# CompVis/unsupervised-part-segmentation

Measured on AMD Instinct MI355X. Metric: images/sec training (CUB 128x128, 10 parts), higher is better.
Workload: dtype bf16

## Files before the change

unsupervised-part-segmentation_amd/csrc/conv_wgrad.hip:

```cpp
#include "common.h"

namespace {

struct WgK {
    int n, hi, wi, ci, ldi, ci_log, cin_v, ho, wo, co, ldo, in_sy, in_sx, ntaps, act_in, want_bias, in_f16;
    float act_slope;
    unsigned long long tap_off, tap_wi;
    const void* in; const void* dout; float* ws;
    float* bias_direct;
};

__device__ inline int wtap_dy(unsigned long long off, int t) { return (int)((off >> (4 * t + 2)) & 3) - 1; }
__device__ inline int wtap_dx(unsigned long long off, int t) { return (int)((off >> (4 * t)) & 3) - 1; }
__device__ inline int wtap_w(unsigned long long wi, int t) { return (int)((wi >> (4 * t)) & 15); }

constexpr int lds_stride(int row_bytes) {
    return ((row_bytes + 63) / 128) * 128 + 64;
}

typedef __attribute__((address_space(3))) s16x4 lds_s16x4;

__device__ inline bf16x8 tr_frag(const unsigned char* tile, int rs, int k0, int c0, int lane) {
    const int g = lane >> 4, i = lane & 15, h = g >> 1;
    const int cb = c0 + 16 * (g & 1), q = i >> 2, pp = i & 3;
    const unsigned char* a0 = tile + (k0 + 8 * h + q) * rs + (cb + 4 * pp) * 2;
    s16x4 lo = __builtin_amdgcn_ds_read_tr16_b64_v4i16((lds_s16x4*)a0);
    s16x4 hi = __builtin_amdgcn_ds_read_tr16_b64_v4i16((lds_s16x4*)(a0 + 4 * rs));
    union { s16x4 s[2]; bf16x8 b; } u;
    u.s[0] = lo; u.s[1] = hi;
    return u.b;
}

template <typename T, int BMW, int BNW>
__global__ __launch_bounds__(256) void conv_wgrad_kernel(const WgK p, const int M, const int cit, const int cot,
                                                         const int chunks_total, const int chunks_per) {
    constexpr int EPC = Chunk<T>::N;
    constexpr int PK = 4 * EPC;
    constexpr int RSA = lds_stride(BMW * (int)sizeof(T));
    constexpr int RSB = lds_stride(BNW * (int)sizeof(T));
    constexpr int NBM = BMW / 32, NBN = BNW / 32;
    constexpr int WM = NBM >= 2 ? ((NBN == 1 && NBM == 4) ? 4 : 2) : 1;
    constexpr int WN = NBN >= 2 ? ((NBM == 1 && NBN == 4) ? 4 : 2) : 1;
    constexpr int TM = NBM / WM, TN = NBN / WN;
    constexpr int ACTIVE = WM * WN;
    constexpr int CPA = BMW / EPC;
    constexpr int CPB = BNW / EPC;
    constexpr int NA = (PK * CPA + 255) / 256;
    constexpr int NB = (PK * CPB + 255) / 256;
    constexpr int BPARTS = 256 / BNW;

    __shared__ __attribute__((aligned(16))) unsigned char smem[PK * (RSA + RSB)];
    unsigned char* Xs = smem;
    unsigned char* Ds = smem + PK * RSA;

    const int tid = threadIdx.x, lane = tid & 63, wid = tid >> 6;
    const float act_ns = ups_slope_eff(p.act_in, p.act_slope);
    const int cot_i = blockIdx.x % cot, cit_i = blockIdx.x / cot;
    const int split = blockIdx.y;
    const int wm = wid / WN, wn = wid % WN;

    const T* __restrict__ in = (const T*)p.in;
    const T* __restrict__ dout = (const T*)p.dout;
    const int hw_o = p.ho * p.wo;
    const int V = p.ntaps * p.ci;
    const int v0 = cit_i * BMW, co0 = cot_i * BNW;
    const bool do_bias = p.want_bias && cit_i == 0;

    const int c_begin = split * chunks_per;
    const int c_end = min(chunks_total, c_begin + chunks_per);

    int xrow0 = 0, xrow1 = 0, xc0 = -1, xc1 = -1, xdy0 = 0, xdx0 = 0, xdy1 = 0, xdx1 = 0;
    {
        auto dec = [&](int idx, int& row, int& c, int& dy, int& dx) {
            c = -1;
            if (idx < PK * CPA) {
                row = idx / CPA;
                const int v = v0 + (idx - row * CPA) * EPC;
                if (v < V) {
                    const int tap = v / p.ci;
                    c = v - tap * p.ci;
                    dy = wtap_dy(p.tap_off, tap); dx = wtap_dx(p.tap_off, tap);
                }
            }
        };
        dec(tid, xrow0, xc0, xdy0, xdx0);
        if (NA > 1) dec(tid + 256, xrow1, xc1, xdy1, xdx1);
    }

    uint4 xa0, xa1, db0, db1;
    const uint4 zero4 = make_uint4(0u, 0u, 0u, 0u);

    auto load_x = [&](int chunk_idx, int row, int c, int dy, int dx) -> uint4 {
        uint4 v = zero4;
        const int m = chunk_idx * PK + row;
        if (c >= 0 && m < M) {
            const int img = m / hw_o, rem = m - img * hw_o;
            const int i = rem / p.wo, j = rem - i * p.wo;
            const int y = i * p.in_sy + dy, x = j * p.in_sx + dx;
            if ((unsigned)y < (unsigned)p.hi && (unsigned)x < (unsigned)p.wi)
                v = *(const uint4*)(in + (((long long)img * p.hi + y) * p.wi + x) * p.ldi + c);
        }
        return v;
    };
    auto load_d = [&](int chunk_idx, int idx) -> uint4 {
        uint4 v = zero4;
        if (idx < PK * CPB) {
            const int row = idx / CPB, cc = idx - row * CPB;
            const int m = chunk_idx * PK + row;
            const int ch = co0 + cc * EPC;
            if (m < M && ch < p.ldo) v = *(const uint4*)(dout + (long long)m * p.ldo + ch);
        }
        return v;
    };
    auto act_u4 = [&](uint4 u) -> uint4 {
        if constexpr (__is_same(T, bf16)) {
            if (p.in_f16) return ups_act_chunk_f16_to_bf16(u, act_ns, p.act_in != UPS_ACT_NONE);
        }
        if (p.act_in != UPS_ACT_NONE) {
            u = ups_act_chunk(u, act_ns, (T*)nullptr);
        }
        return u;
    };
    auto load_chunk = [&](int chunk_idx) {
        xa0 = load_x(chunk_idx, xrow0, xc0, xdy0, xdx0);
        if (NA > 1) xa1 = load_x(chunk_idx, xrow1, xc1, xdy1, xdx1);
        db0 = load_d(chunk_idx, tid);
        if (NB > 1) db1 = load_d(chunk_idx, tid + 256);
    };
    auto stage_chunk = [&]() {
        if (tid < PK * CPA) { const int row = tid / CPA, cc = tid - row * CPA; *(uint4*)(Xs + row * RSA + cc * 16) = act_u4(xa0); }
        if (NA > 1) { const int idx = tid + 256, row = idx / CPA, cc = idx - row * CPA; *(uint4*)(Xs + row * RSA + cc * 16) = act_u4(xa1); }
        if (tid < PK * CPB) { const int row = tid / CPB, cc = tid - row * CPB; *(uint4*)(Ds + row * RSB + cc * 16) = db0; }
        if (NB > 1) { const int idx = tid + 256, row = idx / CPB, cc = idx - row * CPB; *(uint4*)(Ds + row * RSB + cc * 16) = db1; }
    };

    f32x16 acc[TM][TN];
#pragma unroll
    for (int i = 0; i < TM; ++i)
#pragma unroll
        for (int j = 0; j < TN; ++j)
#pragma unroll
            for (int e = 0; e < 16; ++e) acc[i][j][e] = 0.f;
    float bsum = 0.f;
    const int bcol = tid % BNW, bpart = tid / BNW;

    if (c_begin < c_end) load_chunk(c_begin);
    for (int c = c_begin; c < c_end; ++c) {
        stage_chunk();
        __syncthreads();
        if (c + 1 < c_end) load_chunk(c + 1);
        if (do_bias) {
#pragma unroll
            for (int k = 0; k < PK / BPARTS; ++k)
                bsum += ld_as_float<T>((const T*)(Ds + (bpart * (PK / BPARTS) + k) * RSB) + bcol);
        }
        if (wid < ACTIVE) {
            if constexpr (sizeof(T) == 2) {
#pragma unroll
                for (int ks = 0; ks < 2; ++ks) {
                    bf16x8 a[TM], bb[TN];
#pragma unroll
                    for (int i = 0; i < TM; ++i) a[i] = tr_frag(Xs, RSA, ks * 16, (wm * TM + i) * 32, lane);
#pragma unroll
                    for (int j = 0; j < TN; ++j) bb[j] = tr_frag(Ds, RSB, ks * 16, (wn * TN + j) * 32, lane);
#pragma unroll
                    for (int i = 0; i < TM; ++i)
#pragma unroll
                        for (int j = 0; j < TN; ++j)
                            acc[i][j] = __builtin_amdgcn_mfma_f32_32x32x16_bf16(a[i], bb[j], acc[i][j], 0, 0, 0);
                }
            } else {
                const int r = lane & 31, h = lane >> 5;
#pragma unroll
                for (int kk = 0; kk < 8; ++kk) {
                    float a[TM], bb[TN];
#pragma unroll
                    for (int i = 0; i < TM; ++i) a[i] = *(const float*)(Xs + (8 * h + kk) * RSA + ((wm * TM + i) * 32 + r) * 4);
#pragma unroll
                    for (int j = 0; j < TN; ++j) bb[j] = *(const float*)(Ds + (8 * h + kk) * RSB + ((wn * TN + j) * 32 + r) * 4);
#pragma unroll
                    for (int i = 0; i < TM; ++i)
#pragma unroll
                        for (int j = 0; j < TN; ++j)
                            acc[i][j] = __builtin_amdgcn_mfma_f32_32x32x2f32(a[i], bb[j], acc[i][j], 0, 0, 0);
                }
            }
        }
        __syncthreads();
    }

    const long long slab_sz = (long long)p.ntaps * p.cin_v * p.co + p.co;
    float* slab = p.ws + (long long)split * slab_sz;
    if (wid < ACTIVE) {
#pragma unroll
        for (int tn = 0; tn < TN; ++tn) {
            const int col = co0 + (wn * TN + tn) * 32 + (lane & 31);
            if (col >= p.co) continue;
#pragma unroll
            for (int tm = 0; tm < TM; ++tm)
#pragma unroll
                for (int e = 0; e < 16; ++e) {
                    const int v = v0 + (wm * TM + tm) * 32 + (e & 3) + 8 * (e >> 2) + 4 * (lane >> 5);
                    if (v < V) {
                        const int tap = v / p.ci, cch = v - tap * p.ci;
                        if (cch < p.ci_log)
                            slab[((long long)wtap_w(p.tap_wi, tap) * p.cin_v + cch) * p.co + col] = acc[tm][tn][e];
                    }
                }
        }
    }
    if (do_bias) {
        float* red = (float*)smem;
        red[tid] = bsum;
        __syncthreads();
        if (tid < BNW && co0 + tid < p.co) {
            float s = 0.f;
#pragma unroll
            for (int k = 0; k < BPARTS; ++k) s += red[k * BNW + tid];
            if (p.bias_direct) p.bias_direct[co0 + tid] = s;
            else slab[(long long)p.ntaps * p.cin_v * p.co + co0 + tid] = s;
        }
    }
}

__global__ __launch_bounds__(256) void wgrad_reduce_kernel(const float* __restrict__ ws, float* __restrict__ grad,
                                                           float* __restrict__ gbias, int splitk, int ntaps_w, int cin_v,
                                                           int ci_log, int co, long long slab) {
    __shared__ float red[8][32];
    const long long nw = (long long)ntaps_w * ci_log * co;
    const long long total = nw + (gbias ? co : 0);
    const int o = threadIdx.x & 31, g = threadIdx.x >> 5;
    for (long long base = (long long)blockIdx.x * 32; base < total; base += (long long)gridDim.x * 32) {
        const long long idx = base + o;
        const bool ok = idx < total;
        long long off = 0;
        float* dst = nullptr;
        if (ok) {
            if (idx < nw) {
                const int c = (int)(idx % co);
                const long long tr = idx / co;
                const int row = (int)(tr % ci_log), tap = (int)(tr / ci_log);
                off = ((long long)tap * cin_v + row) * co + c;
                dst = grad + off;
            } else {
                off = (long long)ntaps_w * cin_v * co + (idx - nw);
                dst = gbias + (idx - nw);
            }
        }
        float s0 = 0.f, s1 = 0.f, s2 = 0.f, s3 = 0.f;
        if (ok) {
            int k = g;
            for (; k + 24 < splitk; k += 32) {
                s0 += ws[(long long)k * slab + off]; s1 += ws[(long long)(k + 8) * slab + off];
                s2 += ws[(long long)(k + 16) * slab + off]; s3 += ws[(long long)(k + 24) * slab + off];
            }
            for (; k < splitk; k += 8) s0 += ws[(long long)k * slab + off];
        }
        red[g][o] = (s0 + s1) + (s2 + s3);
        __syncthreads();
        if (g == 0 && ok) {
            float t = red[0][o];
#pragma unroll
            for (int q = 1; q < 8; ++q) t += red[q][o];
            *dst = t;
        }
        __syncthreads();
    }
}

template <typename T, int BMW, int BNW>
void launch_tile(const WgK& k, int M, int splitk, hipStream_t s) {
    constexpr int PK = 4 * Chunk<T>::N;
    const int cit = ups_cdiv(k.ntaps * k.ci, BMW), cot = ups_cdiv(k.co, BNW);
    const int chunks_total = ups_cdiv(M, PK);
    const int chunks_per = ups_cdiv(chunks_total, splitk);
    hipLaunchKernelGGL((conv_wgrad_kernel<T, BMW, BNW>), dim3(cit * cot, splitk), dim3(256), 0, s, k, M, cit, cot,
                       chunks_total, chunks_per);
}

template <typename T, int BMW>
void launch_n(const WgK& k, int M, int splitk, hipStream_t s) {
    if (k.co > 64) launch_tile<T, BMW, 128>(k, M, splitk, s);
    else if (k.co > 32) launch_tile<T, BMW, 64>(k, M, splitk, s);
    else launch_tile<T, BMW, 32>(k, M, splitk, s);
}

int tile_of(int c) { return c > 64 ? 128 : (c > 32 ? 64 : 32); }

template <typename T>
void launch_m(const WgK& k, int M, int splitk, hipStream_t s) {
    const int bm = tile_of(k.ntaps * k.ci);
    if (bm == 128) launch_n<T, 128>(k, M, splitk, s);
    else if (bm == 64) launch_n<T, 64>(k, M, splitk, s);
    else launch_n<T, 32>(k, M, splitk, s);
}

int plan_splitk(const ups_wgrad_desc* d) {
    const long long M = (long long)d->n * d->ho * d->wo;
    const int pk = d->dtype == UPS_BF16 ? 32 : 16;
    const int v = d->ntaps * d->ci;
    const int tiles = ups_cdiv(v, tile_of(v)) * ups_cdiv(d->co, tile_of(d->co));
    const int chunks = ups_cdiv(M, pk);
    int sk = ups_cdiv(2048, tiles);
    const int max_by_work = chunks / 8 > 0 ? chunks / 8 : 1;
    if (sk > max_by_work) sk = max_by_work;
    if (sk > 512) sk = 512;
    if (sk < 1) sk = 1;
    return sk;
}

}

int ups_wgrad3x3_plan(const ups_wgrad_desc* d, int* splitk, int* slabs);
int ups_wgrad3x3_run(const ups_wgrad_desc* d, hipStream_t s);
int ups_wgrad3x3_f8_plan(const ups_wgrad_desc* d, int* splitk, int* slabs);
int ups_wgrad3x3_f8_run(const ups_wgrad_desc* d, hipStream_t s);

extern "C" int ups_conv_wgrad_plan(const ups_wgrad_desc* d, int32_t* splitk, size_t* workspace_bytes) {
    UPS_CHECK_ARG(d && splitk && workspace_bytes);
    UPS_CHECK_ARG(d->ntaps >= 1 && d->ntaps <= 9 && d->ci > 0 && d->co > 0);
    int sk3 = 0, slabs3 = 0;
    if (ups_wgrad3x3_f8_plan(d, &sk3, &slabs3) == 0 ||
        ups_wgrad3x3_plan(d, &sk3, &slabs3) == 0) {
        *splitk = sk3;
        *workspace_bytes = (size_t)slabs3 * ((size_t)d->ntaps * d->cin_v * d->co + d->co) * sizeof(float);
        return UPS_OK;
    }
    const int sk = plan_splitk(d);
    *splitk = sk;
    *workspace_bytes = (size_t)sk * ((size_t)d->ntaps * d->cin_v * d->co + d->co) * sizeof(float);
    return UPS_OK;
}

extern "C" int ups_conv_wgrad(const ups_wgrad_desc* d, void* stream) {
    UPS_CHECK_ARG(d != nullptr);
    UPS_CHECK_ARG(d->dtype == UPS_F32 || d->dtype == UPS_BF16);
    UPS_CHECK_ARG(d->in && d->dout && d->grad && d->workspace);
    UPS_CHECK_ARG(d->ci > 0 && d->ci % 8 == 0 && d->ldi % 8 == 0 && d->ci <= d->ldi && d->ldo % 8 == 0);
    UPS_CHECK_ARG(d->ci_log >= 1 && d->ci_log <= d->ci && d->cin_v >= d->ci_log);
    UPS_CHECK_ARG(d->ntaps >= 1 && d->ntaps <= 9 && d->splitk >= 1);
    UPS_CHECK_ARG(d->act_slope >= 0.f && d->act_slope <= 1.f);
    UPS_CHECK_ARG(((uintptr_t)d->in & 15) == 0 && ((uintptr_t)d->dout & 15) == 0);
    const long long M = (long long)d->n * d->ho * d->wo;
    UPS_CHECK_ARG(M > 0 && M <= 0x7fffffffLL);
    WgK k;
    k.n = d->n; k.hi = d->hi; k.wi = d->wi; k.ci = d->ci; k.ldi = d->ldi; k.ci_log = d->ci_log; k.cin_v = d->cin_v;
    k.ho = d->ho; k.wo = d->wo; k.co = d->co; k.ldo = d->ldo; k.in_sy = d->in_sy; k.in_sx = d->in_sx;
    k.ntaps = d->ntaps; k.act_in = d->act_in; k.act_slope = d->act_slope; k.want_bias = d->grad_bias != nullptr;
    k.in_f16 = d->in_f16;
    UPS_CHECK_ARG(!d->in_f16 || (d->dtype == UPS_BF16 && !d->mask_bits));
    k.in = d->in; k.dout = d->dout; k.ws = d->workspace; k.bias_direct = nullptr;
    k.tap_off = 0; k.tap_wi = 0;
    int max_tw = 0;
    for (int t = 0; t < d->ntaps; ++t) {
        UPS_CHECK_ARG(d->tap_dy[t] >= -1 && d->tap_dy[t] <= 2 && d->tap_dx[t] >= -1 && d->tap_dx[t] <= 2);
        UPS_CHECK_ARG(d->tap_w[t] >= 0 && d->tap_w[t] <= 15);
        k.tap_off |= (unsigned long long)(((d->tap_dy[t] + 1) << 2) | (d->tap_dx[t] + 1)) << (4 * t);
        k.tap_wi |= (unsigned long long)d->tap_w[t] << (4 * t);
        if (d->tap_w[t] > max_tw) max_tw = d->tap_w[t];
    }
    UPS_CHECK_ARG(max_tw < d->ntaps);
    hipStream_t s = (hipStream_t)stream;
    int nslabs = d->splitk;
    int sk3 = 0, slabs3 = 0;
    if (d->mask_bits) {
        UPS_CHECK_ARG(d->mask_batch > 0 && d->n % d->mask_batch == 0 && d->n / d->mask_batch <= 32);
        if (ups_wgrad3x3_plan(d, &sk3, &slabs3) != 0) {
            ups_set_error("ups_conv_wgrad: the part-masked form needs the bf16 3x3 / stride-1 patch kernel (16-aligned images)");
            return UPS_E_UNSUPPORTED;
        }
    }
    if (ups_wgrad3x3_f8_plan(d, &sk3, &slabs3) == 0) {
        UPS_CHECK_ARG(d->splitk == sk3 && d->dout_f8_scale && d->in_f8_scale && ((uintptr_t)d->dout_f8 & 15) == 0);
        if (ups_wgrad3x3_f8_run(d, s) != UPS_OK) { ups_set_error("ups_conv_wgrad: fp8 kernel launch setup failed"); return UPS_E_LAUNCH; }
        nslabs = slabs3;
    } else if (ups_wgrad3x3_plan(d, &sk3, &slabs3) == 0) {
        UPS_CHECK_ARG(d->splitk == sk3);
        if (ups_wgrad3x3_run(d, s) != UPS_OK) { ups_set_error("ups_conv_wgrad: patch kernel launch setup failed"); return UPS_E_LAUNCH; }
        nslabs = slabs3;
    } else {
        static int direct = -1;
        if (direct < 0) { const char* e = getenv("UPS_WGRAD_DIRECT"); direct = (e && e[0] == '0') ? 0 : 1; }
        const bool one = direct && d->splitk == 1;
        if (one) { k.ws = d->grad; k.bias_direct = d->grad_bias; }
        if (d->dtype == UPS_F32) launch_m<float>(k, (int)M, d->splitk, s);
        else launch_m<bf16>(k, (int)M, d->splitk, s);
        UPS_LAUNCH_CHECK();
        if (one) return UPS_OK;
    }
    UPS_LAUNCH_CHECK();
    const long long slab = (long long)d->ntaps * d->cin_v * d->co + d->co;
    const long long total = (long long)d->ntaps * d->ci_log * d->co + d->co;
    hipLaunchKernelGGL(wgrad_reduce_kernel, dim3(ups_cdiv(total, 32) > 8192 ? 8192 : ups_cdiv(total, 32)), dim3(256), 0,
                       s, d->workspace, d->grad, d->grad_bias, nslabs, d->ntaps, d->cin_v, d->ci_log, d->co, slab);
    UPS_LAUNCH_CHECK();
    return UPS_OK;
}
```

unsupervised-part-segmentation_amd/switches.py:

```python
import os
from collections import OrderedDict

SWITCHES = OrderedDict([
    ("UPS_LIB", ("", "ab", "lib.py", "path of the library to load instead of csrc/libupsparts_hip.so (A/B builds: tools/ab_build.sh)")),
    ("UPS_DIST_BACKEND", ("nccl", "product", "runner.py", "torch.distributed backend (nccl = RCCL; gloo for the CPU / one-GPU tests)")),
    ("UPS_GRAPH", ("0", "product", "model.py", "1: HIP-graph replay of the step (config key hip_graph)")),
    ("UPS_STREAM_PLAN", ("auto", "product", "model.py", "full | compact | auto: side-stream budget (config key stream_plan; DESIGN section 7)")),
    ("UPS_NO_OVERLAP", ("0", "ab", "ops.py", "1: everything on one stream (per-kernel profiles without CU sharing)")),
    ("UPS_POST_ACT", ("1", "ab", "nets.py", "0: activation-on-load everywhere instead of post-activation storage (config key post_activation_storage)")),
    ("UPS_SIGN_BITS", ("1", "ab", "ops.py", "0: input gradients read the forward input for act' instead of the producer's sign bytes")),
    ("UPS_VGG_FP8", ("0", "ab", "model.py", "1: fp8 copies through the perceptual trunk (config key vgg_fp8; measured slower, DESIGN 3b)")),
    ("UPS_F8_WGRAD", ("1", "ab", "ops.py", "0: bf16 weight gradients in precision fp8")),
    ("UPS_F8_PRODUCER", ("1", "ab", "ops.py", "0: fp8 copies converted by a separate pass instead of the producing epilogue")),
    ("UPS_TOWERS", ("1", "ab", "ops.py", "0: the critics' towers through the generic convolution path instead of the grouped launches")),
    ("UPS_STATE_KERNEL", ("1", "ab", "model.py", "0: the Lagrangian / EMA state update as ~30 torch launches instead of one kernel")),
    ("UPS_LATE_JOIN", ("1", "ab", "model.py", "0: a single rank joins the weight-gradient stream at every segment boundary")),
    ("UPS_EARLY_ADAM", ("1", "ab", "model.py", "0: every key's Adam at the end of the step instead of behind its weight gradients")),
    ("UPS_EARLY_ALPHA", ("1", "ab", "model.py", "0: the appearance code after the pose encoder instead of beside it on `aux`")),
    ("UPS_CRITIC_STREAMS", ("1", "ab", "model.py", "0: the three critics on one stream")),
    ("UPS_COORD_STREAM", ("1", "ab", "ops.py", "0: the CoordConv rows of the weight gradients on the weight-gradient stream itself")),
    ("UPS_NO_D2S", ("0", "ab", "ops.py", "1: the stride-2 layers' input gradient as four phase launches instead of one depth-to-space launch")),
    ("UPS_DP_SIDE_LAUNCH", ("1", "ab", "model.py", "0: bucket all-reduces launched from the launching stream (it then waits for the weight gradients)")),
    ("UPS_DP_STANDIN", ("0", "debug", "dist.py", "1: every bucket all-reduce replaced by a device copy on its own stream (one-GPU stream-budget probe)")),
    ("UPS_FORCE_COLLECTIVES", ("0", "test", "dist.py", "1: issue the collectives at world size 1 (the RCCL call pattern test)")),
    ("UPS_JOIN_TIMING", ("0", "debug", "model.py", "1: HIP events around the end-of-backward joins (tools/probes/join_wait.py)")),
    ("UPS_ROWS_KERNEL", ("1", "test", "conv3x3_rows.hip", "0: row-stream layers through the patch / generic kernels; force: also at small batches (parity tests)")),
    ("UPS_S2_KERNEL", ("1", "ab", "conv3x3_s2.hip", "0: the other stride-2 forwards through the generic kernel")),
    ("UPS_THIN_SW", ("32", "ab", "conv3x3_rows.hip", "16: 16-column strips in the logit convolution (measured equal)")),
    ("UPS_FIRST_LAYER", ("1", "ab", "conv3x3_first.hip", "0: the 3-channel first layers through the generic kernel")),
    ("UPS_FORCE_GENERIC_CONV", ("0", "test", "conv_igemm.hip", "1: every convolution through the generic gather kernel")),
    ("UPS_IGEMM_FORCE", ("", "test", "conv_igemm.hip", "tile variant of the generic kernel")),
    ("UPS_NO_SPLITK", ("0", "ab", "conv_igemm.hip", "1: no split-K for the small-grid generic launches")),
    ("UPS_NO_SMALL_PATCH", ("0", "ab", "conv3x3_patch.hip", "1: no small-tile patch instances")),
    ("UPS_PATCH_CST", ("", "ab", "conv3x3_patch.hip", "patch kernel: constant-stride instances on / off")),
    ("UPS_PATCH_DMA", ("1", "ab", "conv3x3_patch.hip", "0: register-staged patches instead of LDS-DMA")),
    ("UPS_PATCH_MID", ("", "ab", "conv3x3_patch.hip", "patch kernel: mid-size tile selection")),
    ("UPS_PATCH_OCC", ("", "ab", "conv3x3_patch.hip", "patch kernel: blocks per CU override")),
    ("UPS_PATCH_RAGGED", ("1", "ab", "conv3x3_patch.hip", "0: images that are not a multiple of 16 leave the patch kernel")),
    ("UPS_PATCH_STATIC", ("", "ab", "conv3x3_patch.hip", "patch kernel: static-geometry instances on / off")),
    ("UPS_PATCH_THIN128", ("", "ab", "conv3x3_patch.hip", "patch kernel: thin 128-wide instance selection")),
    ("UPS_PATCH_THINOUT", ("", "ab", "conv3x3_patch.hip", "patch kernel: thin-output instance selection")),
    ("UPS_RES_PATCH", ("1", "ab", "conv3x3_patch.hip", "0: the forward's residual from global memory instead of the resident patch")),
    ("UPS_RES_PATCH_DGRAD", ("1", "ab", "conv3x3_patch.hip", "0: the input gradient's residual and sign bytes fetched in the epilogue instead of from the resident patch (round 6)")),
    ("UPS_F8_SCALED", ("1", "ab", "conv3x3_patch.hip", "0: K = 32 fp8 MFMA instead of the block-scaled K = 128 form")),
    ("UPS_WGRAD_DIRECT", ("1", "ab", "conv_wgrad.hip", "0: single-split weight gradients through a slab + reduce launch")),
    ("UPS_WGRAD_SLIDE", ("1", "ab", "conv_wgrad3x3.hip", "0: the plain form of the 3x3 weight gradient (3 % slower step)")),
    ("UPS_PRIOR_PX", ("1", "ab", "priors.hip", "0: the staged prior kernels at P = 10 instead of the pixel-per-lane rings")),
    ("UPS_PRIOR_PX_BPI", ("", "test", "priors.hip", "cap on blocks per image of the pixel-per-lane prior kernels (multi-tile loops at three images)")),
    ("UPS_PRIOR_DIRECT", ("1", "ab", "priors.hip", "0: the staged prior kernels at P = 16 / 20 / 25 instead of the chunk-per-lane direct-from-global forms (round 6)")),
    ("UPS_SOFTMAX_PX", ("1", "ab", "partpath.hip", "0: the LDS-walking soft-max kernel at P = 10")),
    ("UPS_MOMENTS_PX", ("1", "ab", "partpath.hip", "0: the slab form of the spatial moments at P = 10")),
    ("UPS_MOMENTS_PX_BLOCKS", ("", "test", "partpath.hip", "blocks of the pixel-per-lane moments kernel")),
    ("UPS_UNPOOL_MFMA", ("1", "test", "partpath.hip", "0: the VALU form of unpool_bwd (the unit test compares both)")),
])

COMPILE_TIME = ("UPS_ABLATE_BARRIER", "UPS_ABLATE_PATCHWAIT", "UPS_ABLATE_WWAIT", "UPS_EPI_PRIO", "UPS_ABLATE_DMA", "UPS_ABLATE_EPI", "UPS_ABLATE_GLOAD", "UPS_ABLATE_LSTORE", "UPS_ABLATE_MFMA", "UPS_F8S_WN1", "UPS_OCC2_FRAG2",
                "UPS_PATCH_A2", "UPS_PHASE_TIMING", "UPS_W8_NO_DMA", "UPS_W8_NO_MFMA", "UPS_W8_NO_QUANT", "UPS_W8_NO_XLOAD", "UPS_WGRAD_NO_PIPE",
                "UPS_ROWS_FWD_SIGN", "UPS_ROWS_NO_FENCE", "UPS_VMAX_BUILTIN")
NOT_SWITCHES = ("UPS_ABI_VERSION", "UPS_ACT_", "UPS_OK", "UPS_E_", "UPS_BF16", "UPS_F16", "UPS_F32", "UPS_CHECK_ARG", "UPS_LAUNCH_CHECK")


def value(name):
    return os.environ.get(name, SWITCHES[name][0])


def flag(name):
    d = SWITCHES[name][0]
    v = os.environ.get(name, d)
    return v != "0" if d == "1" else v == "1"


def report():
    diff = ["{}={}".format(k, os.environ[k]) for k, (d, _, _, _) in SWITCHES.items() if k in os.environ and os.environ[k] != d]
    return "UPS switches: " + (", ".join(diff) if diff else "all defaults")
```

Baseline: 2108.

## Add phase-split LDS patch kernel for stride-2 3x3 weight gradients

Adds a dedicated weight-gradient kernel for 3x3 stride-2 bf16 convolutions. It stages a polyphase-decomposed input patch and a swizzled dout tile in double-buffered LDS, reads them with transpose reads, and feeds 32x32x16 MFMAs, with each wave covering three taps. This replaces the generic split-K kernel for those layers and is meant to cut redundant global loads and im2col overhead. The kernel is limited to narrow outputs (co <= 64, wo <= 64) and can be disabled with a new switch.

Result: no change. 2117 (median of 6 runs) (+0.4%).

```diff
diff --git a/unsupervised-part-segmentation_amd/csrc/conv_wgrad.hip b/unsupervised-part-segmentation_amd/csrc/conv_wgrad.hip
--- a/unsupervised-part-segmentation_amd/csrc/conv_wgrad.hip
+++ b/unsupervised-part-segmentation_amd/csrc/conv_wgrad.hip
@@ -315,6 +315,8 @@
 int ups_wgrad3x3_run(const ups_wgrad_desc* d, hipStream_t s);
 int ups_wgrad3x3_f8_plan(const ups_wgrad_desc* d, int* splitk, int* slabs);
 int ups_wgrad3x3_f8_run(const ups_wgrad_desc* d, hipStream_t s);
+bool ups_wgrad3x3_s2_eligible(const ups_wgrad_desc* d);
+int ups_wgrad3x3_s2_run(const ups_wgrad_desc* d, float* ws, float* bias_direct, hipStream_t s);
 
 extern "C" int ups_conv_wgrad_plan(const ups_wgrad_desc* d, int32_t* splitk, size_t* workspace_bytes) {
     UPS_CHECK_ARG(d && splitk && workspace_bytes);
@@ -383,7 +385,12 @@
         if (direct < 0) { const char* e = getenv("UPS_WGRAD_DIRECT"); direct = (e && e[0] == '0') ? 0 : 1; }
         const bool one = direct && d->splitk == 1;
         if (one) { k.ws = d->grad; k.bias_direct = d->grad_bias; }
-        if (d->dtype == UPS_F32) launch_m<float>(k, (int)M, d->splitk, s);
+        if (ups_wgrad3x3_s2_eligible(d)) {
+            if (ups_wgrad3x3_s2_run(d, k.ws, k.bias_direct, s) != UPS_OK) {
+                ups_set_error("ups_conv_wgrad: stride-2 patch kernel launch setup failed");
+                return UPS_E_LAUNCH;
+            }
+        } else if (d->dtype == UPS_F32) launch_m<float>(k, (int)M, d->splitk, s);
         else launch_m<bf16>(k, (int)M, d->splitk, s);
         UPS_LAUNCH_CHECK();
         if (one) return UPS_OK;
diff --git a/unsupervised-part-segmentation_amd/csrc/conv_wgrad3x3_s2.hip b/unsupervised-part-segmentation_amd/csrc/conv_wgrad3x3_s2.hip
--- /dev/null
+++ b/unsupervised-part-segmentation_amd/csrc/conv_wgrad3x3_s2.hip
@@ -0,0 +1,274 @@
+#include <stdlib.h>
+
+#include "common.h"
+
+namespace {
+
+constexpr int CB = 32;
+constexpr int RSX = 64;
+constexpr int PK = 32;
+
+struct WgS2K {
+    int hi, wi, ho, wo, ci, ldi, ci_log, cin_v, co, ldo, act_in, want_bias, in_f16;
+    int M, chunks_per, th, plc, plp;
+    float act_slope;
+    int trow[9];
+    unsigned long long tap_wi;
+    const void* in; const void* dout; float* ws;
+    float* bias_direct;
+};
+
+typedef __attribute__((address_space(3))) s16x4 lds_s2_s16x4;
+
+__device__ inline bf16x8 tr_frag_x(const unsigned char* tile, int row0, int lane) {
+    const int g = lane >> 4, i = lane & 15, h = g >> 1;
+    const int cb = 16 * (g & 1), q = i >> 2, pp = i & 3;
+    const unsigned char* a0 = tile + (row0 + 8 * h + q) * RSX + (cb + 4 * pp) * 2;
+    s16x4 lo = __builtin_amdgcn_ds_read_tr16_b64_v4i16((lds_s2_s16x4*)a0);
+    s16x4 hi = __builtin_amdgcn_ds_read_tr16_b64_v4i16((lds_s2_s16x4*)(a0 + 4 * RSX));
+    union { s16x4 s[2]; bf16x8 b; } u;
+    u.s[0] = lo; u.s[1] = hi;
+    return u.b;
+}
+
+template <int BN> __device__ __forceinline__ int ds_swz(int row) {
+    if constexpr (BN == 64) return (row >> 1) & 1;
+    else return 0;
+}
+template <int BN> __device__ __forceinline__ int d_off(int row, int col) {
+    return row * (BN * 2) + (((col >> 5) ^ ds_swz<BN>(row)) << 6) + (col & 31) * 2;
+}
+
+template <int BN>
+__device__ inline bf16x8 tr_frag_dout(const unsigned char* tile, int row0, int wco, int lane) {
+    constexpr int RS = BN * 2;
+    const int g = lane >> 4, i = lane & 15, h = g >> 1, q = i >> 2, pp = i & 3;
+    const int row = row0 + 8 * h + q;
+    const unsigned char* a0 = tile + row * RS + ((wco ^ ds_swz<BN>(row)) << 6) + 32 * (g & 1) + 8 * pp;
+    s16x4 lo = __builtin_amdgcn_ds_read_tr16_b64_v4i16((lds_s2_s16x4*)a0);
+    s16x4 hi = __builtin_amdgcn_ds_read_tr16_b64_v4i16((lds_s2_s16x4*)(a0 + 4 * RS));
+    union { s16x4 s[2]; bf16x8 b; } u;
+    u.s[0] = lo; u.s[1] = hi;
+    return u.b;
+}
+
+template <int BN> struct S2Geo {
+    static constexpr int WCO = BN / 32;
+    static constexpr int NWC = 3 * WCO;
+    static constexpr int NW = NWC < 4 ? 4 : NWC;
+    static constexpr int NT = 64 * NW;
+    static constexpr int SPX = 128;
+    static constexpr int XMAX = 4 * 3 * 65;
+    static constexpr int NX = (XMAX * 4 + NT - 1) / NT;
+    static constexpr int ND = (SPX * BN / 8 + NT - 1) / NT;
+    static constexpr int XB = XMAX * RSX, DB = SPX * BN * 2;
+    static constexpr int BPARTS = 256 / BN;
+};
+
+template <int BN>
+__global__ __launch_bounds__(S2Geo<BN>::NT) void conv_wgrad3x3_s2_kernel(const WgS2K p, const int cot) {
+    using G = S2Geo<BN>;
+    constexpr int NT = G::NT, NX = G::NX, ND = G::ND, SPX = G::SPX, CPD = BN / 8;
+    extern __shared__ __attribute__((aligned(16))) unsigned char smem[];
+    unsigned char* Xbuf = smem;
+    unsigned char* Dbuf = smem + 2 * G::XB;
+
+    const int tid = threadIdx.x, lane = tid & 63;
+    const int wid = __builtin_amdgcn_readfirstlane(tid >> 6);
+    const float act_ns = ups_slope_eff(p.act_in, p.act_slope);
+    const int cot_i = blockIdx.x % cot, cit_i = blockIdx.x / cot, split = blockIdx.y;
+    const int ci0 = cit_i * CB, co0 = cot_i * BN;
+    const bf16* __restrict__ in = (const bf16*)p.in;
+    const bf16* __restrict__ dout = (const bf16*)p.dout;
+    const bool do_bias = p.want_bias && cit_i == 0;
+    const bool cwave = wid < G::NWC;
+    const int w_co = wid % G::WCO, w_t0 = 3 * (wid / G::WCO);
+
+    const int m_beg = split * p.chunks_per * PK;
+    const int m_end = min(p.M, m_beg + p.chunks_per * PK);
+    const int hw_o = p.ho * p.wo;
+    const int st_beg = m_beg / SPX, st_end = m_beg < m_end ? (m_end + SPX - 1) / SPX : st_beg;
+
+    const int nxi = 4 * p.plp * 4;
+    unsigned xrc[NX], xs[NX];
+#pragma unroll
+    for (int k = 0; k < NX; ++k) {
+        const int item = min(tid + NT * k, nxi - 1);
+        const int pix = item >> 2, cc = item & 3;
+        const int pl = pix / p.plp, rem = pix - pl * p.plp;
+        const int a = rem / p.plc, b = rem - a * p.plc;
+        const int r = 2 * a + (pl >> 1), c = 2 * b + (pl & 1);
+        xrc[k] = (tid + NT * k < nxi && ci0 + cc * 8 < p.ci) ? (unsigned)((r << 8) | c) : 0xffffu;
+        xs[k] = (unsigned)(pix * RSX + cc * 16);
+    }
+    unsigned dsrc[ND], dslot[ND];
+#pragma unroll
+    for (int k = 0; k < ND; ++k) {
+        const int item = min(tid + NT * k, SPX * CPD - 1);
+        const int row = item / CPD, s = item - row * CPD;
+        dsrc[k] = (unsigned)(row * p.ldo + min(co0 + s * 8, p.ldo - 8));
+        dslot[k] = (unsigned)d_off<BN>(row, s * 8);
+    }
+
+    uint4 rx[NX], rd[ND];
+    unsigned rxok = 0u;
+    const uint4 zero4 = make_uint4(0u, 0u, 0u, 0u);
+
+    auto load_step = [&](int st) __attribute__((always_inline)) {
+        const int m0 = st * SPX;
+        const int img = m0 / hw_o, i0 = (m0 - img * hw_o) / p.wo;
+        const int y0 = 2 * i0 - 1;
+        const bf16* ib = in + (long long)img * p.hi * p.wi * p.ldi + ci0;
+#pragma unroll
+        for (int k = 0; k < NX; ++k) {
+            unsigned rc = xrc[k];
+            asm volatile("" : "+v"(rc));
+            const int y = y0 + (int)(rc >> 8), x = (int)(rc & 0xffu) - 1;
+            const bool ok = rc != 0xffffu && (unsigned)y < (unsigned)p.hi && (unsigned)x < (unsigned)p.wi;
+            const bf16* src = ok ? ib + ((long long)y * p.wi + x) * p.ldi + (xs[k] & 48u) / 2 : in;
+            rx[k] = *(const uint4*)src;
+            rxok = ok ? rxok | (1u << k) : rxok & ~(1u << k);
+        }
+        const bf16* db = dout + (long long)m0 * p.ldo;
+#pragma unroll
+        for (int k = 0; k < ND; ++k) rd[k] = *(const uint4*)(db + dsrc[k]);
+    };
+    auto store_step = [&](int buf) __attribute__((always_inline)) {
+        unsigned char* X = Xbuf + buf * G::XB;
+#pragma unroll
+        for (int k = 0; k < NX; ++k) {
+            uint4 v = (rxok >> k) & 1u ? rx[k] : zero4;
+            if (p.in_f16) v = ups_act_chunk_f16_to_bf16(v, act_ns, p.act_in != UPS_ACT_NONE);
+            else if (p.act_in != UPS_ACT_NONE) v = ups_act_chunk(v, act_ns, (bf16*)nullptr);
+            if (tid + NT * k < nxi) *(uint4*)(X + xs[k]) = v;
+        }
+        unsigned char* D = Dbuf + buf * G::DB;
+#pragma unroll
+        for (int k = 0; k < ND; ++k)
+            if (tid + NT * k < SPX * CPD) *(uint4*)(D + dslot[k]) = rd[k];
+    };
+
+    f32x16 acc[3];
+#pragma unroll
+    for (int t = 0; t < 3; ++t)
+#pragma unroll
+        for (int e = 0; e < 16; ++e) acc[t][e] = 0.f;
+    int trow[3];
+#pragma unroll
+    for (int t = 0; t < 3; ++t) trow[t] = p.trow[min(w_t0 + t, 8)];
+    float bsum = 0.f;
+    const int bcol = tid % BN, bpart = tid / BN;
+    const int gpr = p.wo / 16;
+
+    if (st_beg < st_end) { load_step(st_beg); store_step(0); }
+    __syncthreads();
+    for (int st = st_beg; st < st_end; ++st) {
+        const int buf = (st - st_beg) & 1;
+        if (st + 1 < st_end) load_step(st + 1);
+        const unsigned char* X = Xbuf + buf * G::XB;
+        const unsigned char* D = Dbuf + buf * G::DB;
+        const int m0 = st * SPX;
+        const int g_lo = max(0, (m_beg - m0) / 16), g_hi = min(SPX / 16, (m_end - m0) / 16);
+        if (cwave) {
+            for (int g = g_lo; g < g_hi; ++g) {
+                const int ks = g / gpr, j0 = (g - ks * gpr) * 16;
+                const bf16x8 b = tr_frag_dout<BN>(D, g * 16, w_co, lane);
+#pragma unroll
+                for (int t = 0; t < 3; ++t) {
+                    const bf16x8 a = tr_frag_x(X, trow[t] + ks * p.plc + j0, lane);
+                    acc[t] = __builtin_amdgcn_mfma_f32_32x32x16_bf16(a, b, acc[t], 0, 0, 0);
+                }
+            }
+        }
+        if (do_bias && tid < 256) {
+            for (int ch = g_lo / 2; ch < g_hi / 2; ++ch)
+#pragma unroll
+                for (int k = 0; k < PK / G::BPARTS; ++k)
+                    bsum += (float)*(const bf16*)(D + d_off<BN>(ch * PK + bpart * (PK / G::BPARTS) + k, bcol));
+        }
+        if (st + 1 < st_end) store_step(buf ^ 1);
+        __syncthreads();
+    }
+
+    float* slab = p.ws + (long long)split * ((long long)9 * p.cin_v * p.co + p.co);
+    const int col = co0 + w_co * 32 + (lane & 31);
+    if (cwave && col < p.co) {
+#pragma unroll
+        for (int t = 0; t < 3; ++t) {
+            const int tw = (int)((p.tap_wi >> (4 * (w_t0 + t))) & 15);
+#pragma unroll
+            for (int e = 0; e < 16; ++e) {
+                const int row = ci0 + (e & 3) + 8 * (e >> 2) + 4 * (lane >> 5);
+                if (row < p.ci_log) slab[((long long)tw * p.cin_v + row) * p.co + col] = acc[t][e];
+            }
+        }
+    }
+    if (do_bias) {
+        float* red = (float*)smem;
+        if (tid < 256) red[tid] = bsum;
+        __syncthreads();
+        if (tid < BN && co0 + tid < p.co) {
+            float s = 0.f;
+#pragma unroll
+            for (int k = 0; k < G::BPARTS; ++k) s += red[k * BN + tid];
+            if (p.bias_direct) p.bias_direct[co0 + tid] = s;
+            else slab[(long long)9 * p.cin_v * p.co + co0 + tid] = s;
+        }
+    }
+}
+
+int pick_bn(const ups_wgrad_desc* d) { return d->co > 64 ? 128 : (d->co > 32 ? 64 : 32); }
+
+template <int BN>
+int launch_s2(const WgS2K& k, int cit, int cot, int splitk, hipStream_t s) {
+    using G = S2Geo<BN>;
+    const size_t shmem = 2 * (size_t)(G::XB + G::DB);
+    static UpsPerDevice attr_set;
+    if (!attr_set) {
+        if (hipFuncSetAttribute((const void*)conv_wgrad3x3_s2_kernel<BN>, hipFuncAttributeMaxDynamicSharedMemorySize,
+                                (int)shmem) != hipSuccess) return UPS_E_LAUNCH;
+        attr_set = true;
+    }
+    hipLaunchKernelGGL((conv_wgrad3x3_s2_kernel<BN>), dim3(cit * cot, splitk), dim3(G::NT), shmem, s, k, cot);
+    return UPS_OK;
+}
+
+}
+
+bool ups_wgrad3x3_s2_eligible(const ups_wgrad_desc* d) {
+    if (d->dtype != UPS_BF16 || d->ntaps != 9 || d->in_sy != 2 || d->in_sx != 2 || d->mask_bits || d->in_f8_scale) return false;
+    if (pick_bn(d) == 128) return false;
+    const int spx = 128;
+    if (d->wo % 16 || d->wo > 64 || d->ho % (spx / d->wo) || d->ldo < 8) return false;
+    if ((long long)d->n * d->ho * d->wo > 0x7fffffffLL || (long long)spx * d->ldo >= (1ll << 31)) return false;
+    for (int t = 0; t < 9; ++t) {
+        if (d->tap_dy[t] < -1 || d->tap_dy[t] > 2 || d->tap_dx[t] < -1 || d->tap_dx[t] > 2) return false;
+        if (d->tap_w[t] < 0 || d->tap_w[t] > 8) return false;
+    }
+    const char* e = getenv("UPS_WGRAD_PATCH_S2");
+    if (e && e[0] == '0') return false;
+    const char* force = getenv("UPS_FORCE_GENERIC_CONV");
+    return !(force && force[0] == '1');
+}
+
+int ups_wgrad3x3_s2_run(const ups_wgrad_desc* d, float* ws, float* bias_direct, hipStream_t s) {
+    const int bn = pick_bn(d);
+    const int spx = 128;
+    WgS2K k;
+    k.hi = d->hi; k.wi = d->wi; k.ho = d->ho; k.wo = d->wo; k.ci = d->ci; k.ldi = d->ldi; k.ci_log = d->ci_log;
+    k.cin_v = d->cin_v; k.co = d->co; k.ldo = d->ldo; k.act_in = d->act_in; k.act_slope = d->act_slope;
+    k.want_bias = d->grad_bias != nullptr; k.in_f16 = d->in_f16;
+    k.M = d->n * d->ho * d->wo;
+    k.chunks_per = ups_cdiv(ups_cdiv(k.M, PK), d->splitk);
+    k.th = spx / d->wo; k.plc = d->wo + 1; k.plp = (k.th + 1) * k.plc;
+    k.in = d->in; k.dout = d->dout; k.ws = ws; k.bias_direct = bias_direct;
+    k.tap_wi = 0;
+    for (int t = 0; t < 9; ++t) {
+        const int ry = d->tap_dy[t] + 1, rx = d->tap_dx[t] + 1;
+        k.trow[t] = ((ry & 1) * 2 + (rx & 1)) * k.plp + (ry >> 1) * k.plc + (rx >> 1);
+        k.tap_wi |= (unsigned long long)d->tap_w[t] << (4 * t);
+    }
+    const int cit = ups_cdiv(d->ci, CB), cot = ups_cdiv(d->co, bn);
+    if (bn == 64) return launch_s2<64>(k, cit, cot, d->splitk, s);
+    return launch_s2<32>(k, cit, cot, d->splitk, s);
+}
diff --git a/unsupervised-part-segmentation_amd/switches.py b/unsupervised-part-segmentation_amd/switches.py
--- a/unsupervised-part-segmentation_amd/switches.py
+++ b/unsupervised-part-segmentation_amd/switches.py
@@ -44,6 +44,7 @@
     ("UPS_RES_PATCH_DGRAD", ("1", "ab", "conv3x3_patch.hip", "0: the input gradient's residual and sign bytes fetched in the epilogue instead of from the resident patch (round 6)")),
     ("UPS_F8_SCALED", ("1", "ab", "conv3x3_patch.hip", "0: K = 32 fp8 MFMA instead of the block-scaled K = 128 form")),
     ("UPS_WGRAD_DIRECT", ("1", "ab", "conv_wgrad.hip", "0: single-split weight gradients through a slab + reduce launch")),
+    ("UPS_WGRAD_PATCH_S2", ("1", "ab", "conv_wgrad3x3_s2.hip", "0: the 3x3 / stride-2 weight gradients through the generic split-K kernel")),
     ("UPS_WGRAD_SLIDE", ("1", "ab", "conv_wgrad3x3.hip", "0: the plain form of the 3x3 weight gradient (3 % slower step)")),
     ("UPS_PRIOR_PX", ("1", "ab", "priors.hip", "0: the staged prior kernels at P = 10 instead of the pixel-per-lane rings")),
     ("UPS_PRIOR_PX_BPI", ("", "test", "priors.hip", "cap on blocks per image of the pixel-per-lane prior kernels (multi-tile loops at three images)")),
```
